# skokec/DAU-ConvNet

Measured on AMD Instinct MI355X. Metric: DAU fwd+bwd GSamples/s (N*H*W/s), higher is better.
Workload: dtype f32

## Files before the change

dau-convnet_amd/csrc/k_dense_split.hip:

```cpp
#include <algorithm>
#include <cstdint>
#include <cstdlib>
#include <type_traits>

#include "dau_tiled.hpp"

#ifndef DAU_SPLIT_R
#define DAU_SPLIT_R 3
#endif
#ifndef DAU_SPLIT_NS
#define DAU_SPLIT_NS s3
#endif

namespace dau {
namespace DAU_SPLIT_NS {

typedef _Float16 f16x8 __attribute__((ext_vector_type(8)));
typedef __attribute__((ext_vector_type(16))) float f32x16;
typedef __attribute__((ext_vector_type(4))) unsigned u32x4;
typedef __attribute__((address_space(3))) void* lds_ptr_t;
typedef __attribute__((address_space(1))) const void* glb_ptr_t;

namespace {

constexpr int kDR = DAU_SPLIT_R;
constexpr int kDK = 2 * kDR + 1;
constexpr int kDSpan = kDK - 1;
constexpr int kDTaps = kDK * kDK;
constexpr int kDRows = 8;
constexpr int kDFB = 128;
constexpr int kAhead = 2;
#ifndef DAU_SPLIT_FLUSH_TAPS
#define DAU_SPLIT_FLUSH_TAPS 0
#endif
constexpr int kFlushTaps = DAU_SPLIT_FLUSH_TAPS > 0 ? DAU_SPLIT_FLUSH_TAPS : kDK;
#ifndef DAU_SPLIT_FLUSH_ROWS
#define DAU_SPLIT_FLUSH_ROWS 4
#endif
constexpr int kFlushRows = DAU_SPLIT_FLUSH_ROWS;

inline size_t round_up(size_t v, size_t a) { return (v + a - 1) / a * a; }

struct SplitScales {
    unsigned max_w_bits;
    float sw, inv_sw;
    float pad[5];
};
__host__ __device__ __forceinline__ const float* scales_sx(const SplitScales* sc) { return reinterpret_cast<const float*>(sc + 1); }
__host__ __device__ __forceinline__ const float* scales_inv_sx(const SplitScales* sc, int N) { return reinterpret_cast<const float*>(sc + 1) + N; }
constexpr int kPartials = 1024;
inline int absmax_groups_per_image(int N, long per) {
    const long fit = std::max(1, kPartials / N), want = (per / 4 + 255) / 256 + 1;
    return (int)std::min(fit, want);
}
inline size_t scales_bytes(int N) { return sizeof(SplitScales) + (size_t)2 * N * sizeof(float); }

constexpr int kMaxSub = 4;
struct SplitGeom {
    int sub;
    int nsub_a, nb_a, nsub_b, nb_b;
    int nrb8, nrb4;
    int tall;
    int Hs, Ws, nchunk, CoutP;
    size_t hdr_bytes, xs_bytes, ws_bytes;
};

SplitGeom split_geometry(const DenseConfig& c) {
    SplitGeom g{};
    g.sub = (c.W + 7) / 8;
    const int nblocks = (g.sub + kMaxSub - 1) / kMaxSub, base = g.sub / nblocks, rem = g.sub % nblocks;
    if (rem) { g.nsub_a = base + 1; g.nb_a = rem; g.nsub_b = base; g.nb_b = nblocks - rem; }
    else { g.nsub_a = base; g.nb_a = nblocks; g.nsub_b = 0; g.nb_b = 0; }
    const int left = c.H % kDRows;
    const long wgs = (long)c.N * ((c.H + kDRows - 1) / kDRows) * nblocks * ((c.Cout + kDFB - 1) / kDFB);
    const int rows4 = DAU_TUNE_INT("DAU_SPLIT_ROWS4", 1);
    g.nrb4 = (left >= 1 && left <= 4 && rows4 != 0 && (wgs >= 1024 || rows4 == 2)) ? 1 : 0;
    g.nrb8 = c.H / kDRows + (left && !g.nrb4 ? 1 : 0);
    g.Hs = g.nrb8 * kDRows + g.nrb4 * 4 + kDSpan;
    {
        const int t4 = (c.W + 3) / 4;
        const long rows8 = (long)g.nrb8 * kDRows;
        const long flat = (long)(g.nrb4 ? rows8 + 4 : (c.H + 3) / 4 * 4) * g.sub * 8;
        const long tall = rows8 * t4 * 4 + (g.nrb4 ? 4L * g.sub * 8 : 0);
        const int want = DAU_TUNE_INT("DAU_SPLIT_TALL", 1);
        g.tall = (want != 0 && g.nrb8 > 0 && (t4 == 5 || t4 == 7) && (tall * 20 <= flat * 19 || want == 2)) ? t4 : 0;
    }
    g.Ws = g.sub * 8 + kDSpan;
    g.nchunk = (c.Cin + 15) / 16;
    g.CoutP = (int)round_up(c.Cout, kDFB);
    g.hdr_bytes = round_up(scales_bytes(c.N) + (size_t)2 * (kPartials + c.N) * sizeof(unsigned), 256);
    g.xs_bytes = round_up((size_t)c.N * g.nchunk * 4 * g.Hs * g.Ws * 16 + 4096, 256);
    g.ws_bytes = round_up(((size_t)g.nchunk * kDTaps + 8) * 2 * g.CoutP * 32, 256);
    return g;
}

constexpr int lds_pitch(int nsub) {
    int p = nsub * 8 + kDSpan;
    while (p % 16 != 8) ++p;
    return p;
}
constexpr int lds_pitch_narrow(int ntiles) {
    int p = ntiles * 4 + kDSpan;
    while (p % 16 != 4 && p % 16 != 12) ++p;
    return p;
}

}

__device__ __forceinline__ unsigned finite_bits(unsigned b) { return b < 0x7f800000u ? b : 0u; }

__device__ __forceinline__ long absmax_head(const void* p, long per, int elem_bytes, int vec_bytes) {
    const uintptr_t a = reinterpret_cast<uintptr_t>(p);
    if (a % elem_bytes) return per;
    const long head = (long)((vec_bytes - a % vec_bytes) % vec_bytes) / elem_bytes;
    return head < per ? head : per;
}

__global__ void __launch_bounds__(256) split_absmax_kernel(const float* __restrict__ in, long per, int gpi, int act, const UnitRef* __restrict__ table,
                                                           long units, unsigned* __restrict__ partial, int cap, const Guard guard) {
    if (!guard_pass(guard)) return;
    unsigned mx = 0, mw = 0;
    const int n = blockIdx.x / gpi, j = blockIdx.x - n * gpi;
    const long stride = (long)gpi * blockDim.x, t0 = j * (long)blockDim.x + threadIdx.x;
    if (act == kActF16) {
        auto wide = [](unsigned h) { return finite_bits(__float_as_uint(f16_bits_to_float(h)) & 0x7fffffffu); };
        const unsigned short* e = reinterpret_cast<const unsigned short*>(in) + n * per;
        const long head = absmax_head(e, per, 2, 8), n4 = (per - head) / 4;
        const uint2* p = reinterpret_cast<const uint2*>(e + head);
        for (long i = t0; i < n4; i += stride) {
            const uint2 v = p[i];
            mx = max(mx, max(max(wide(v.x & 0xffffu), wide(v.x >> 16)), max(wide(v.y & 0xffffu), wide(v.y >> 16))));
        }
        for (long i = t0; i < per - n4 * 4; i += stride) mx = max(mx, wide(e[i < head ? i : i + n4 * 4]));
    } else if (act == kActBF16) {
        const unsigned short* e = reinterpret_cast<const unsigned short*>(in) + n * per;
        const long head = absmax_head(e, per, 2, 8), n4 = (per - head) / 4;
        const uint2* p = reinterpret_cast<const uint2*>(e + head);
        for (long i = t0; i < n4; i += stride) {
            const uint2 v = p[i];
            mx = max(mx, max(max(finite_bits((v.x << 16) & 0x7fffffffu), finite_bits(v.x & 0x7fff0000u)),
                             max(finite_bits((v.y << 16) & 0x7fffffffu), finite_bits(v.y & 0x7fff0000u))));
        }
        for (long i = t0; i < per - n4 * 4; i += stride) mx = max(mx, finite_bits(((unsigned)e[i < head ? i : i + n4 * 4] << 16) & 0x7fffffffu));
    } else {
        const float* e = in + n * per;
        const long head = absmax_head(e, per, 4, 16), n4 = (per - head) / 4;
        const uint4* p = reinterpret_cast<const uint4*>(e + head);
        for (long i = t0; i < n4; i += stride) {
            const uint4 v = p[i];
            mx = max(mx, max(max(finite_bits(v.x & 0x7fffffffu), finite_bits(v.y & 0x7fffffffu)),
                             max(finite_bits(v.z & 0x7fffffffu), finite_bits(v.w & 0x7fffffffu))));
        }
        for (long i = t0; i < per - n4 * 4; i += stride) mx = max(mx, finite_bits(__float_as_uint(e[i < head ? i : i + n4 * 4]) & 0x7fffffffu));
    }
    for (long u = blockIdx.x * (long)blockDim.x + threadIdx.x; u < units; u += (long)gridDim.x * blockDim.x) {
        const UnitRef r = table[u];
        mw = max(mw, finite_bits(__float_as_uint(fabsf(r.w00) + fabsf(r.w01) + fabsf(r.w10) + fabsf(r.w11))));
    }
    __shared__ unsigned sx[4], sw[4];
    for (int m = 32; m >= 1; m >>= 1) { mx = max(mx, (unsigned)__shfl_xor((int)mx, m)); mw = max(mw, (unsigned)__shfl_xor((int)mw, m)); }
    if ((threadIdx.x & 63) == 0) { sx[threadIdx.x >> 6] = mx; sw[threadIdx.x >> 6] = mw; }
    __syncthreads();
    if (threadIdx.x == 0) {
        partial[blockIdx.x] = max(max(sx[0], sx[1]), max(sx[2], sx[3]));
        partial[cap + blockIdx.x] = max(max(sw[0], sw[1]), max(sw[2], sw[3]));
    }
}

__device__ __forceinline__ float limb_scale(float m) {
    if (!(m > 0.0f) || !(m < INFINITY)) return 1.0f;
    int e = ilogbf(m);
    e = 13 - e;
    e = e > 100 ? 100 : (e < -100 ? -100 : e);
    return ldexpf(1.0f, e);
}

__global__ void __launch_bounds__(256) split_scales_kernel(const unsigned* __restrict__ partial, int N, int gpi, int cap, int G,
                                                           SplitScales* __restrict__ out, const Guard guard) {
    if (!guard_pass(guard)) return;
    const int n = blockIdx.x;
    const unsigned* src = n < N ? partial + (long)n * gpi : partial + cap;
    const int cnt = n < N ? gpi : N * gpi;
    unsigned m = 0;
    for (int i = threadIdx.x; i < cnt; i += 256) m = max(m, src[i]);
    __shared__ unsigned sm[4];
    for (int k = 32; k >= 1; k >>= 1) m = max(m, (unsigned)__shfl_xor((int)m, k));
    if ((threadIdx.x & 63) == 0) sm[threadIdx.x >> 6] = m;
    __syncthreads();
    if (threadIdx.x == 0) {
        m = max(max(sm[0], sm[1]), max(sm[2], sm[3]));
        float* sx = reinterpret_cast<float*>(out + 1);
        if (n < N) {
            const float s = limb_scale(__uint_as_float(m));
            sx[n] = s; sx[N + n] = 1.0f / s;
        } else {
            const float s = limb_scale(__uint_as_float(m) * (float)G);
            out->max_w_bits = m; out->sw = s; out->inv_sw = 1.0f / s;
        }
    }
}

constexpr int kScT = 64;
__global__ void __launch_bounds__(kScT) split_densify_kernel(const UnitRef* __restrict__ table, int Cin, int G, int Cout, int CoutP, int nchunk,
                                                             const SplitScales* __restrict__ sc, _Float16* __restrict__ wsd, const Guard guard) {
    __shared__ float acc[kDTaps * kScT];
    if (!guard_pass(guard)) return;
    constexpr int FPB = kScT / 16;
    const int tid = threadIdx.x, sl = tid & 15;
    const int fq = blockIdx.x % (CoutP / FPB), chunk = blockIdx.x / (CoutP / FPB);
    const int f = fq * FPB + (tid >> 4), c = chunk * 16 + sl;
#pragma unroll 7
    for (int tap = 0; tap < kDTaps; ++tap) acc[tap * kScT + tid] = 0.0f;
    if (c < Cin && f < Cout) {
        for (int g = 0; g < G; ++g) {
            const UnitRef u = table[((long)c * G + g) * Cout + f];
            const int ty = u.oy + kDR, tx = u.ox + kDR;
            const bool y0 = ty >= 0 && ty < kDK, y1 = ty + 1 >= 0 && ty + 1 < kDK, x0 = tx >= 0 && tx < kDK, x1 = tx + 1 >= 0 && tx + 1 < kDK;
            if (y0 && x0) acc[(ty * kDK + tx) * kScT + tid] += u.w00;
            if (y0 && x1) acc[(ty * kDK + tx + 1) * kScT + tid] += u.w01;
            if (y1 && x0) acc[((ty + 1) * kDK + tx) * kScT + tid] += u.w10;
            if (y1 && x1) acc[((ty + 1) * kDK + tx + 1) * kScT + tid] += u.w11;
        }
    }
    const float sw = sc->sw;
    _Float16* dst = wsd + ((long)chunk * kDTaps * 2 * CoutP + f) * 16 + sl;
    const long limb = (long)CoutP * 16, tapstride = 2 * limb;
#pragma unroll 7
    for (int tap = 0; tap < kDTaps; ++tap) {
        const float v = acc[tap * kScT + tid] * sw;
        const _Float16 hi = (_Float16)v;
        dst[tap * tapstride] = hi;
        dst[tap * tapstride + limb] = (_Float16)(v - (float)hi);
    }
}

constexpr int kSP = 80;
struct SplitStageArgs {
    const float* in;
    const float* taps;
    const SplitScales* sc;
    _Float16* xs;
    int N, C, H, W, mirrored;
    int Hs, Ws, nchunk;
    int RB, nbands, nsegs;
    int vec;
    Guard guard;
};

__device__ __forceinline__ int fast_div(int i, int d, float inv) {
    int q = (int)(((float)i + 0.5f) * inv);
    const int r = i - q * d;
    q += (r >= d) - (r < 0);
    return q;
}

template <int K, int NCH>
__device__ __forceinline__ void split_stage_rows(float* rawl, const float* px, int col, int ch0, int wave, int nw, int lh, int ncols) {
    constexpr int kr = (K - 1) / 2;
    if (col >= ncols) return;
    float gx[K];
#pragma unroll
    for (int j = 0; j < K; ++j) gx[j] = px[j];
    for (int r = wave; r < lh; r += nw) {
        float* row = rawl + (r * 8 + ch0) * kSP + 8 + col;
        float acc[NCH];
#pragma unroll
        for (int ch = 0; ch < NCH; ++ch) {
            acc[ch] = 0.0f;
#pragma unroll
            for (int i = 0; i < K; ++i) acc[ch] = fmaf(row[ch * kSP + i - kr], gx[i], acc[ch]);
        }
#pragma unroll
        for (int ch = 0; ch < NCH; ++ch) row[ch * kSP] = acc[ch];
    }
}

template <int K, int NCH>
__device__ __forceinline__ void split_stage_walk(const float* rawl, const float* py, float sx, int col, int ch0, int ya, int yb,
                                                 int y0, int x0, int x1, int Ws, u32x4* xhi, u32x4* xlo) {
    constexpr int kr = (K - 1) / 2;
    const int x = x0 + col;
    if (x >= x1) return;
    float gy[K];
#pragma unroll
    for (int j = 0; j < K; ++j) gy[j] = py[j];
    float ring[K][NCH];
    const int nin = yb - ya + 2 * kr;
    char* dhi = reinterpret_cast<char*>(xhi + (long)kDR * Ws + kDR + x) + ch0 * 2;
    char* dlo = reinterpret_cast<char*>(xlo + (long)kDR * Ws + kDR + x) + ch0 * 2;
    for (int s0 = 0; s0 < nin; s0 += K) {
#pragma unroll
        for (int j = 0; j < K; ++j) {
            const int s = s0 + j;
            if (s < nin) {
                const float* row = rawl + ((ya - y0 + s) * 8 + ch0) * kSP + 8 + col;
#pragma unroll
                for (int ch = 0; ch < NCH; ++ch) ring[j][ch] = row[ch * kSP];
                if (s >= K - 1) {
                    typedef _Float16 f16xn __attribute__((ext_vector_type(NCH)));
                    f16xn oh, ol;
#pragma unroll
                    for (int ch = 0; ch < NCH; ++ch) {
                        float acc = 0.0f;
#pragma unroll
                        for (int i = 0; i < K; ++i) acc = fmaf(ring[(j + 1 + i) % K][ch], gy[i], acc);
                        acc *= sx;
                        const _Float16 hi = (_Float16)acc;
                        oh[ch] = hi;
                        ol[ch] = (_Float16)(acc - (float)hi);
                    }
                    const long o = (long)(ya + s - (K - 1)) * Ws * 16;
                    *reinterpret_cast<f16xn*>(dhi + o) = oh;
                    *reinterpret_cast<f16xn*>(dlo + o) = ol;
                }
            }
        }
    }
}

#ifndef DAU_SPLIT_STAGE_THREADS
#define DAU_SPLIT_STAGE_THREADS 512
#endif
constexpr int kStageThreads = DAU_SPLIT_STAGE_THREADS;
template <int KN, int A>
__global__ void __launch_bounds__(kStageThreads) split_stage_kernel(const SplitStageArgs a) {
    constexpr int K = KN & (kNhwcArg - 1);
    constexpr bool NHWC = (KN & kNhwcArg) != 0;
    extern __shared__ __attribute__((aligned(16))) float rawl[];
    if (!guard_pass(a.guard)) return;
    constexpr int kr = (K - 1) / 2;
    constexpr int PPR = kSP / 4;
    const int lane = threadIdx.x & 63, wave = threadIdx.x >> 6, nw = blockDim.x >> 6;
    int t = blockIdx.x;
    const int seg = t % a.nsegs; t /= a.nsegs;
    const int band = t % a.nbands; t /= a.nbands;
    const int grp = t % (2 * a.nchunk);
    const int n = t / (2 * a.nchunk);
    const int y0 = band * a.RB, y1 = y0 + a.RB < a.H ? y0 + a.RB : a.H;
    const int x0 = seg * 64, x1 = x0 + 64 < a.W ? x0 + 64 : a.W;
    const int lh = y1 - y0 + 2 * kr;
    const long plane = (long)a.H * a.W;
    if constexpr (NHWC) {
        constexpr int CPP = A == kActF32 ? 4 : 8, PARTS = 8 / CPP;
        const int pieces = lh * kSP * PARTS;
        constexpr int UB = (13 * 256 + kStageThreads - 1) / kStageThreads;
        for (int i0 = threadIdx.x; i0 < pieces; i0 += kStageThreads * UB) {
            float v[UB][CPP];
#pragma unroll
            for (int u = 0; u < UB; ++u) {
                const int i = i0 + u * kStageThreads, part = i % PARTS, rj = i / PARTS, r = rj / kSP, j = rj - r * kSP;
                const int c = grp * 8 + part * CPP, y = y0 - kr + r, x = x0 - 8 + j;
                const bool pix = y >= 0 && y < a.H && x >= 0 && x < a.W && i < pieces;
                if (a.vec) {
                    const bool ok = pix && c < a.C;
                    const long idx = ok ? nhwc_index(n, c, y, x, a.C, a.H, a.W) : 0;
                    if constexpr (A == kActF32) {
                        const float4 w = *reinterpret_cast<const float4*>(a.in + idx);
                        v[u][0] = mask_act(w.x, ok); v[u][1] = mask_act(w.y, ok); v[u][2] = mask_act(w.z, ok); v[u][3] = mask_act(w.w, ok);
                    } else {
                        const uint4 w = *reinterpret_cast<const uint4*>(reinterpret_cast<const unsigned short*>(a.in) + idx);
                        const unsigned q[4] = {w.x, w.y, w.z, w.w};
#pragma unroll
                        for (int k = 0; k < 4; ++k) {
                            if constexpr (A == kActF16) {
                                v[u][2 * k] = mask_act(f16_bits_to_float(q[k] & 0xffffu), ok);
                                v[u][2 * k + 1] = mask_act(f16_bits_to_float(q[k] >> 16), ok);
                            } else {
                                const unsigned m = ok ? 0xffffffffu : 0u;
                                v[u][2 * k] = __uint_as_float((q[k] << 16) & m);
                                v[u][2 * k + 1] = __uint_as_float(q[k] & 0xffff0000u & m);
                            }
                        }
                    }
                } else {
#pragma unroll
                    for (int k = 0; k < CPP; ++k) {
                        const bool ok = pix && c + k < a.C;
                        v[u][k] = mask_act(load_act_t<A>(a.in, ok ? nhwc_index(n, c + k, y, x, a.C, a.H, a.W) : 0), ok);
                    }
                }
            }
#pragma unroll
            for (int u = 0; u < UB; ++u) {
                const int i = i0 + u * kStageThreads, part = i % PARTS, rj = i / PARTS, r = rj / kSP, j = rj - r * kSP;
                if (i < pieces) {
#pragma unroll
                    for (int k = 0; k < CPP; ++k) rawl[(r * 8 + part * CPP + k) * kSP + j] = v[u][k];
                }
            }
        }
    } else
    {
        const int pieces = lh * 8 * PPR;
        constexpr int UB = (13 * 256 + kStageThreads - 1) / kStageThreads;
        for (int i0 = threadIdx.x; i0 < pieces; i0 += kStageThreads * UB) {
            float4 v[UB];
#pragma unroll
            for (int u = 0; u < UB; ++u) {
                const int i = i0 + u * kStageThreads, rc = i / PPR, q = i - rc * PPR, r = rc >> 3, ch = rc & 7;
                const int c = grp * 8 + ch, y = y0 - kr + r, xs = x0 - 8 + 4 * q;
                const bool row_in = c < a.C && y >= 0 && y < a.H && i < pieces;
                const long base = ((long)n * a.C + (c < a.C ? c : 0)) * plane;
                if (a.vec) {
                    const bool ok = row_in && xs >= 0 && xs + 4 <= a.W;
                    const long idx = base + (ok ? (long)y * a.W + xs : 0);
                    if constexpr (A == kActF16) {
                        const uint2 w = *reinterpret_cast<const uint2*>(reinterpret_cast<const unsigned short*>(a.in) + idx);
                        v[u] = make_float4(mask_act(f16_bits_to_float(w.x & 0xffffu), ok), mask_act(f16_bits_to_float(w.x >> 16), ok),
                                           mask_act(f16_bits_to_float(w.y & 0xffffu), ok), mask_act(f16_bits_to_float(w.y >> 16), ok));
                    } else if constexpr (A == kActBF16) {
                        const uint2 w = *reinterpret_cast<const uint2*>(reinterpret_cast<const unsigned short*>(a.in) + idx);
                        const unsigned m = ok ? 0xffffffffu : 0u;
                        v[u] = make_float4(__uint_as_float((w.x << 16) & m), __uint_as_float(w.x & 0xffff0000u & m),
                                           __uint_as_float((w.y << 16) & m), __uint_as_float(w.y & 0xffff0000u & m));
                    } else {
                        const float4 w = *reinterpret_cast<const float4*>(a.in + idx);
                        v[u] = make_float4(mask_act(w.x, ok), mask_act(w.y, ok), mask_act(w.z, ok), mask_act(w.w, ok));
                    }
                } else {
                    float e[4];
#pragma unroll
                    for (int k = 0; k < 4; ++k) {
                        const bool ok = row_in && xs + k >= 0 && xs + k < a.W;
                        e[k] = mask_act(load_act_t<A>(a.in, base + (ok ? (long)y * a.W + xs + k : 0)), ok);
                    }
                    v[u] = make_float4(e[0], e[1], e[2], e[3]);
                }
            }
#pragma unroll
            for (int u = 0; u < UB; ++u) {
                const int i = i0 + u * kStageThreads;
                if (i < pieces) *reinterpret_cast<float4*>(rawl + (long)i * 4) = v[u];
            }
        }
    }
    const int chunk = grp >> 1, half = grp & 1;
    const long splane = (long)a.Hs * a.Ws;
    u32x4* xhi = reinterpret_cast<u32x4*>(a.xs) + ((((long)n * a.nchunk + chunk) * 2 + 0) * 2 + half) * splane;
    u32x4* xlo = xhi + 2 * splane;
    {
        const int rs0 = band == 0 ? 0 : y0 + kDR, rs1 = band == a.nbands - 1 ? a.Hs : y1 + kDR;
        const int cs0 = seg == 0 ? 0 : x0 + kDR, cs1 = seg == a.nsegs - 1 ? a.Ws : x1 + kDR;
        const int cw = cs1 - cs0, cnt = (rs1 - rs0) * cw;
        const float inv = 1.0f / (float)cw;
        const u32x4 z = {0u, 0u, 0u, 0u};
        for (int i = threadIdx.x; i < cnt; i += blockDim.x) {
            const int rr = fast_div(i, cw, inv), r = rs0 + rr, cc = cs0 + i - rr * cw;
            if (r >= y0 + kDR && r < y1 + kDR && cc >= x0 + kDR && cc < x1 + kDR) continue;
            xhi[(long)r * a.Ws + cc] = z;
            xlo[(long)r * a.Ws + cc] = z;
        }
    }
    __syncthreads();
    const float* px = a.taps + (a.mirrored ? kTapGXR : kTapGX) * kTapPitch;
    const float* py = a.taps + (a.mirrored ? kTapGYR : kTapGY) * kTapPitch;
    if (x1 - x0 <= 32) split_stage_rows<K, 4>(rawl, px, lane & 31, (lane >> 5) * 4, wave, nw, lh, x1 - x0);
    else split_stage_rows<K, 8>(rawl, px, lane, 0, wave, nw, lh, x1 - x0);
    __syncthreads();
    const int SR = (y1 - y0 + nw - 1) / nw;
    const int ya = y0 + wave * SR, yb = ya + SR < y1 ? ya + SR : y1;
    if (ya >= yb) return;
    const float sx = scales_sx(a.sc)[n];
    if (x1 - x0 <= 32) split_stage_walk<K, 4>(rawl, py, sx, lane & 31, (lane >> 5) * 4, ya, yb, y0, x0, x1, a.Ws, xhi, xlo);
    else split_stage_walk<K, 8>(rawl, py, sx, lane, 0, ya, yb, y0, x0, x1, a.Ws, xhi, xlo);
}

struct SplitArgs {
    const _Float16* xs;
    const _Float16* wsd;
    const SplitScales* sc;
    float* out;
    const float* partial;
    int N, Cout, CoutP, H, W, Hs, Ws, nchunk, ncb, nrb, out_act;
    int col0;
    int row0;
    Guard guard;
};

constexpr int kNhwcVecOut = 0x100;
template <int NSUBN, int RG = 2, bool TT = false, bool H16 = false, bool ADD = false>
__global__ void __launch_bounds__(512) split_gather_kernel(const SplitArgs a) {
    constexpr int NSUB = NSUBN & (kNhwcArg - 1);
    constexpr bool NHWC = (NSUBN & kNhwcArg) != 0;
    static_assert(!TT || RG == 2, "tall tiles: blocks of eight rows");
    constexpr int TW = TT ? 4 : 8;
    constexpr int P = TT ? lds_pitch_narrow(NSUB) : lds_pitch(NSUB);
    constexpr int kRowsWG = 4 * RG;
    constexpr int NT0 = (RG == 2 && !TT) ? NSUB : (NSUB + 1) / 2;
    constexpr int NT1 = TT ? NSUB / 2 : NT0;
    constexpr int WR = kRowsWG + kDSpan;
    constexpr int HALF = WR * P * 16;
    constexpr int BUFU = 4 * WR * P;
    constexpr int NPIECE = (BUFU + 63) / 64;
    constexpr int BUF = NPIECE * 1024;
    constexpr int PPW = (NPIECE + 7) / 8;
    extern __shared__ __attribute__((aligned(16))) char smem[];
    if (!guard_pass(a.guard)) return;
    const int lane = threadIdx.x & 63;
    const int wave = __builtin_amdgcn_readfirstlane(threadIdx.x >> 6);
    const int fw = wave & 3, pw = wave >> 2;
    const int prow = (RG == 2 && !TT) ? 4 * pw : 0, ptile = (RG == 2 && !TT) ? 0 : pw * NT0;
    int t;
#ifdef DAU_SPLIT_NO_XCD_MAP
    t = blockIdx.x;
#else
    {
        const int nblk = gridDim.x, xcd = blockIdx.x % 8, idx = blockIdx.x / 8;
        const int per = nblk / 8, rem = nblk % 8;
        t = (xcd < rem ? xcd * (per + 1) : rem * (per + 1) + (xcd - rem) * per) + idx;
    }
#endif
    const int fb = t % (a.CoutP / kDFB); t /= (a.CoutP / kDFB);
    const int cb = t % a.ncb; t /= a.ncb;
    const int rb = t % a.nrb;
    const int n = t / a.nrb;
    const int h = lane >> 5, nn = lane & 31;

    const long xs_plane = (long)a.Hs * a.Ws;
    const int colb = a.col0 + cb * NSUB * TW;
    const int rowb = a.row0 + rb * kRowsWG;
    const u32x4* xsrc = reinterpret_cast<const u32x4*>(a.xs) + ((long)n * a.nchunk * 4) * xs_plane + (long)rowb * a.Ws + colb;
    int goff[PPW];
#pragma unroll
    for (int i = 0; i < PPW; ++i) {
        int piece = wave + 8 * i;
        piece = piece < NPIECE ? piece : NPIECE - 1;
        int L = piece * 64 + lane;
        L = L < BUFU ? L : BUFU - 1;
        const int ph = L / (WR * P), rem = L - ph * (WR * P), r = rem / P, c = rem - r * P;
        goff[i] = (int)(ph * xs_plane + (long)r * a.Ws + c);
    }
    auto issue = [&](int chunk, int buf) {
        const u32x4* src = xsrc + (long)chunk * 4 * xs_plane;
#pragma unroll
        for (int i = 0; i < PPW; ++i) {
            int piece = wave + 8 * i;
            piece = piece < NPIECE ? piece : NPIECE - 1;
            __builtin_amdgcn_global_load_lds((glb_ptr_t)(src + goff[i]), (lds_ptr_t)(smem + buf * BUF + piece * 1024), 16, 0, 0);
        }
    };

    const int prr = TT ? nn >> 2 : nn >> 3, pcc = TT ? nn & 3 : nn & 7;
    float* const out_ptr = a.out;
    const float* const part_ptr = a.partial;
    const bool out_bf16 = NHWC ? (a.out_act & 0xff) != 0 : a.out_act != 0;
    const bool vec_out = NHWC && (a.out_act & kNhwcVecOut) != 0;
    const int out_c = a.Cout, out_h = a.H, out_w = a.W;
    auto body = [&](auto ntc) __attribute__((always_inline)) {
    constexpr int NT = decltype(ntc)::value;
    f32x16 sum[NT], acc[NT];
    f32x16 zero;
#pragma unroll
    for (int i = 0; i < 16; ++i) zero[i] = 0.0f;
#pragma unroll
    for (int j = 0; j < NT; ++j) { sum[j] = zero; acc[j] = zero; }
    int rows_chained = 0;

    const f16x8* wp = reinterpret_cast<const f16x8*>(a.wsd) + ((long)(fb * kDFB + fw * 32 + nn)) * 2 + h;
    const long wlo = (long)a.CoutP * 2, wtap = 2 * wlo;
    const unsigned lane_base = (unsigned)(h * HALF + ((prow + prr) * P + ptile * TW + pcc) * 16);

#ifdef DAU_SPLIT_NO_IDLE_WAVES
    const bool live = true;
#else
    const bool live = rowb + prow < a.H && ptile < NSUB && colb + ptile * TW < a.W && fb * kDFB + fw * 32 < a.Cout;
#endif
    issue(0, 0);
    f16x8 ah[kDK], al[kDK], an[2], bn[2];
    static_assert(kAhead == 2 && kDK >= 5 && kDK <= 9, "the A ring below is written for two taps ahead");
#pragma unroll
    for (int i = 0; i < kAhead; ++i) { ah[i] = wp[i * wtap]; al[i] = wp[i * wtap + wlo]; }
    asm volatile("s_waitcnt vmcnt(0)" ::: "memory");
    __syncthreads();
    for (int chunk = 0; chunk < a.nchunk; ++chunk) {
        const int buf = chunk & 1;
        if (chunk + 1 < a.nchunk) issue(chunk + 1, buf ^ 1);
        const unsigned bbase = lane_base + buf * BUF;
#pragma unroll 1
        for (int ty = 0; ty < (live ? kDK : 0); ++ty) {
            const unsigned brow = bbase + ty * P * 16;
            f16x8 xh[NT], xl[NT];
#pragma unroll
            for (int j = 0; j < NT; ++j) xh[j] = *reinterpret_cast<const f16x8*>(smem + brow + (TW * j) * 16);
#pragma unroll
            for (int tx = 0; tx < kDK; ++tx) {
#pragma unroll
                for (int j = 0; j < NT; ++j) xl[j] = *reinterpret_cast<const f16x8*>(smem + brow + 2 * HALF + (tx + TW * j) * 16);
#pragma unroll
                for (int j = 0; j < NT; ++j) acc[j] = __builtin_amdgcn_mfma_f32_32x32x16_f16(ah[tx], xh[j], (kFlushRows == 1 && tx % kFlushTaps == 0) ? zero : acc[j], 0, 0, 0);
                if (tx + kAhead < kDK) { ah[tx + kAhead] = wp[(tx + kAhead) * wtap]; al[tx + kAhead] = wp[(tx + kAhead) * wtap + wlo]; }
                if (tx == 2 || tx == 3) { an[tx - 2] = wp[(kDK + tx - 2) * wtap]; bn[tx - 2] = wp[(kDK + tx - 2) * wtap + wlo]; }
#pragma unroll
                for (int j = 0; j < NT; ++j) acc[j] = __builtin_amdgcn_mfma_f32_32x32x16_f16(al[tx], xh[j], acc[j], 0, 0, 0);
                if (tx + 1 < kDK) {
#pragma unroll
                    for (int j = 0; j < NT; ++j) xh[j] = *reinterpret_cast<const f16x8*>(smem + brow + (tx + 1 + TW * j) * 16);
                }
#pragma unroll
                for (int j = 0; j < NT; ++j) acc[j] = __builtin_amdgcn_mfma_f32_32x32x16_f16(ah[tx], xl[j], acc[j], 0, 0, 0);
                if (tx == 0) __builtin_amdgcn_sched_group_barrier(0x100, 2 * NT, 0);
                else __builtin_amdgcn_sched_group_barrier(0x100, NT, 0);
                __builtin_amdgcn_sched_group_barrier(0x008, NT, 0);
                if (tx == 2 || tx == 3) __builtin_amdgcn_sched_group_barrier(0x020, 4, 0);
                else if (tx + kAhead < kDK) __builtin_amdgcn_sched_group_barrier(0x020, 2, 0);
                __builtin_amdgcn_sched_group_barrier(0x008, NT, 0);
                if (tx + 1 < kDK) __builtin_amdgcn_sched_group_barrier(0x100, NT, 0);
                __builtin_amdgcn_sched_group_barrier(0x008, NT, 0);
                if ((tx + 1) % kFlushTaps == 0 && tx + 1 < kDK) {
#pragma unroll
                    for (int j = 0; j < NT; ++j) sum[j] += acc[j];
                }
            }
            wp += kDK * wtap;
            ah[0] = an[0]; al[0] = bn[0]; ah[1] = an[1]; al[1] = bn[1];
            if constexpr (kFlushRows == 1) {
#pragma unroll
                for (int j = 0; j < NT; ++j) sum[j] += acc[j];
            } else {
                if (++rows_chained == kFlushRows) {
                    rows_chained = 0;
#pragma unroll
                    for (int j = 0; j < NT; ++j) { sum[j] += acc[j]; acc[j] = zero; }
                }
            }
        }
        if (chunk + 1 < a.nchunk) {
            asm volatile("s_waitcnt vmcnt(0)" ::: "memory");
            __syncthreads();
        }
    }

    if constexpr (kFlushRows > 1) {
#pragma unroll
        for (int j = 0; j < NT; ++j) sum[j] += acc[j];
    }
    const float inv_w = a.sc->inv_sw, inv_x = scales_inv_sx(a.sc, a.N)[n];
    const int y = rowb + prow + prr;
    const long plane = (long)out_h * out_w;
#pragma unroll
    for (int j = 0; j < NT; ++j) {
        const int x = colb + TW * (ptile + j) + pcc;
        if constexpr (NHWC) {
            if (y < out_h && x < out_w && ptile + j < NSUB) {
                const long pix = ((long)n * out_h + y) * out_w + x;
#pragma unroll
                for (int g4 = 0; g4 < 4; ++g4) {
                    const int f0 = fb * kDFB + fw * 32 + 8 * g4 + 4 * h;
                    float v[4];
#pragma unroll
                    for (int k = 0; k < 4; ++k) {
                        if constexpr (ADD) {
                            const int fc = f0 + k < out_c ? f0 + k : out_c - 1;
                            v[k] = sum[j][4 * g4 + k] * inv_w * inv_x + part_ptr[((long)n * out_c + fc) * plane + (long)y * out_w + x];
                        } else {
                            v[k] = sum[j][4 * g4 + k] * inv_w * inv_x;
                        }
                    }
                    const long o = pix * out_c + f0;
                    if (vec_out) {
                        if (f0 < out_c) {
                            if constexpr (H16) {
                                typedef _Float16 f16x4 __attribute__((ext_vector_type(4)));
                                *reinterpret_cast<f16x4*>(reinterpret_cast<unsigned short*>(out_ptr) + o) =
                                    f16x4{(_Float16)v[0], (_Float16)v[1], (_Float16)v[2], (_Float16)v[3]};
                            } else if (out_bf16) {
                                *reinterpret_cast<uint2*>(reinterpret_cast<unsigned short*>(out_ptr) + o) =
                                    make_uint2(bf16_bits(v[0]) | (bf16_bits(v[1]) << 16), bf16_bits(v[2]) | (bf16_bits(v[3]) << 16));
                            } else {
                                *reinterpret_cast<float4*>(out_ptr + o) = make_float4(v[0], v[1], v[2], v[3]);
                            }
                        }
                    } else {
#pragma unroll
                        for (int k = 0; k < 4; ++k) {
                            if (f0 + k < out_c) {
                                if constexpr (H16) store_act_t<kActF16>(out_ptr, o + k, v[k], false);
                                else store_act(out_ptr, o + k, v[k], out_bf16, false);
                            }
                        }
                    }
                }
            }
        } else
        if (y < out_h && x < out_w && ptile + j < NSUB) {
#pragma unroll
            for (int i = 0; i < 16; ++i) {
                const int f = fb * kDFB + fw * 32 + (i & 3) + 8 * (i >> 2) + 4 * h;
                if (f < out_c) {
                    const long o = ((long)n * out_c + f) * plane + (long)y * out_w + x;
                    if constexpr (ADD) {
                        const float v = sum[j][i] * inv_w * inv_x + part_ptr[o];
                        if constexpr (H16) store_act_t<kActF16>(out_ptr, o, v, false);
                        else store_act(out_ptr, o, v, out_bf16, false);
                    } else if constexpr (H16) store_act_t<kActF16>(out_ptr, o, sum[j][i] * inv_w * inv_x, false);
                    else store_act(out_ptr, o, sum[j][i] * inv_w * inv_x, out_bf16, false);
                }
            }
        }
    }
    };
    if constexpr (TT) {
        if (pw == 0) body(std::integral_constant<int, NT0>{});
        else body(std::integral_constant<int, NT1>{});
    } else {
        body(std::integral_constant<int, NT0>{});
    }
}

namespace {

template <int NSUB, int RG, bool TT>
constexpr size_t split_lds_bytes() { return 2 * (size_t)((4 * (4 * RG + kDSpan) * (TT ? lds_pitch_narrow(NSUB) : lds_pitch(NSUB)) + 63) / 64) * 1024; }

template <int NSUB, int RG, bool TT = false>
void launch_split(hipStream_t st, const SplitArgs* a, int grid, bool h16, bool add, bool nhwc) {
    constexpr int NH = NSUB | kNhwcArg;
    auto kern = h16 ? split_gather_kernel<NSUB, RG, TT, true> : split_gather_kernel<NSUB, RG, TT, false>;
    if (nhwc) kern = h16 ? split_gather_kernel<NH, RG, TT, true> : split_gather_kernel<NH, RG, TT, false>;
#if DAU_SPLIT_R == 3
    if (add) kern = h16 ? split_gather_kernel<NSUB, RG, TT, true, true> : split_gather_kernel<NSUB, RG, TT, false, true>;
    if (add && nhwc) kern = h16 ? split_gather_kernel<NH, RG, TT, true, true> : split_gather_kernel<NH, RG, TT, false, true>;
#endif
    if (!a) { (void)hipFuncSetAttribute(reinterpret_cast<const void*>(kern), hipFuncAttributeMaxDynamicSharedMemorySize, 160 * 1024); return; }
    constexpr size_t lds = split_lds_bytes<NSUB, RG, TT>();
    hipLaunchKernelGGL(kern, dim3(grid), dim3(512), lds, st, *a);
}

void dispatch_split(int nsub, int rg, bool h16, hipStream_t st, const SplitArgs* a, int grid, bool tall, bool add, bool nhwc) {
    if (tall) {
        if (nsub == 5) launch_split<5, 2, true>(st, a, grid, h16, add, nhwc);
        else launch_split<7, 2, true>(st, a, grid, h16, add, nhwc);
        return;
    }
    if (rg == 1) {
        switch (nsub) {
            case 1: launch_split<1, 1>(st, a, grid, h16, add, nhwc); break;
            case 2: launch_split<2, 1>(st, a, grid, h16, add, nhwc); break;
            case 3: launch_split<3, 1>(st, a, grid, h16, add, nhwc); break;
            default: launch_split<4, 1>(st, a, grid, h16, add, nhwc); break;
        }
        return;
    }
    switch (nsub) {
        case 1: launch_split<1, 2>(st, a, grid, h16, add, nhwc); break;
        case 2: launch_split<2, 2>(st, a, grid, h16, add, nhwc); break;
        case 3: launch_split<3, 2>(st, a, grid, h16, add, nhwc); break;
        default: launch_split<4, 2>(st, a, grid, h16, add, nhwc); break;
    }
}

const void* stage_for(int blur_k, int act, bool nhwc = false) {
#define DAU_SPLIT_STAGE(K) case K: if (nhwc) return act == kActF16 ? reinterpret_cast<const void*>(split_stage_kernel<K | kNhwcArg, kActF16>) : \
                                          act == kActBF16 ? reinterpret_cast<const void*>(split_stage_kernel<K | kNhwcArg, kActBF16>) : \
                                                            reinterpret_cast<const void*>(split_stage_kernel<K | kNhwcArg, kActF32>); \
                                   return act == kActF16 ? reinterpret_cast<const void*>(split_stage_kernel<K, kActF16>) : \
                                          act == kActBF16 ? reinterpret_cast<const void*>(split_stage_kernel<K, kActBF16>) : \
                                                            reinterpret_cast<const void*>(split_stage_kernel<K, kActF32>)
    switch (blur_k) {
        DAU_SPLIT_STAGE(3);
        DAU_SPLIT_STAGE(5);
        DAU_SPLIT_STAGE(7);
        DAU_SPLIT_STAGE(9);
        DAU_SPLIT_STAGE(11);
        default: return nullptr;
    }
#undef DAU_SPLIT_STAGE
}
void stage_plan(const DenseConfig& c, int* RB, int* nbands, size_t* lds) {
    const int kr = (c.blur_k - 1) / 2;
    int rows = 52 * 1024 / (8 * kSP * 4) - 2 * kr;
    const int rb = DAU_TUNE_INT("DAU_SPLIT_STAGE_RB", 0);
    if (rb > 0) rows = rb;
    rows = rows < 4 ? 4 : rows;
    const int nb = (c.H + rows - 1) / rows;
    *nbands = nb; *RB = (c.H + nb - 1) / nb;
    *lds = (size_t)(*RB + 2 * kr) * 8 * kSP * 4;
}

}

bool split_gather_configure(int N, int Cin, int Cout, int G, int H, int W, int R, int blur_k, int act, DenseConfig* cfg) {
    if (R != kDR || !stage_for(blur_k, act)) return false;
    DenseConfig c{};
    c.N = N; c.Cin = Cin; c.Cout = Cout; c.G = G; c.H = H; c.W = W; c.R = R; c.blur_k = blur_k; c.act = act;
    const SplitGeom g = split_geometry(c);
    c.nsub = g.nsub_a;
    c.ftiles = 1;
    if ((size_t)g.nchunk * 4 * g.Hs * g.Ws > (size_t)1 << 30) return false;
    *cfg = c;
    return true;
}

size_t split_gather_workspace_bytes(const DenseConfig& c) {
    const SplitGeom g = split_geometry(c);
    return g.hdr_bytes + g.xs_bytes + g.ws_bytes;
}

void split_gather_init(const DenseConfig& c) {
    const SplitGeom g = split_geometry(c);
    const bool h16 = c.act == kActF16;
    for (int rg = 1; rg <= 2; ++rg) {
        if (!(rg == 2 ? g.nrb8 : g.nrb4)) continue;
        for (int add = 0; add <= (kDR == 3 ? 1 : 0); ++add) {
            if (rg == 2 && g.tall) { dispatch_split(g.tall, 2, h16, nullptr, nullptr, 0, true, add != 0, c.nhwc != 0); continue; }
            dispatch_split(g.nsub_a, rg, h16, nullptr, nullptr, 0, false, add != 0, c.nhwc != 0);
            if (g.nb_b) dispatch_split(g.nsub_b, rg, h16, nullptr, nullptr, 0, false, add != 0, c.nhwc != 0);
        }
    }
    (void)hipFuncSetAttribute(stage_for(c.blur_k, c.act, c.nhwc != 0), hipFuncAttributeMaxDynamicSharedMemorySize, 160 * 1024);
}

void split_gather_prepare(hipStream_t st, const DenseConfig& c, const float* in, const float* filters, bool mirrored,
                          const UnitRef* table, void* workspace, const Guard& guard) {
    const SplitGeom g = split_geometry(c);
    char* ws = static_cast<char*>(workspace);
    SplitScales* sc = reinterpret_cast<SplitScales*>(ws);
    unsigned* partial = reinterpret_cast<unsigned*>(ws + scales_bytes(c.N));
    _Float16* xs = reinterpret_cast<_Float16*>(ws + g.hdr_bytes);
    _Float16* wsd = reinterpret_cast<_Float16*>(ws + g.hdr_bytes + g.xs_bytes);
    const long per = (long)c.Cin * c.H * c.W, units = (long)c.Cin * c.G * c.Cout;
    const int gpi = absmax_groups_per_image(c.N, per), cap = kPartials + c.N;
    hipLaunchKernelGGL(split_absmax_kernel, dim3(c.N * gpi), dim3(256), 0, st, in, per, gpi, c.act, table, units, partial, cap, guard);
    hipLaunchKernelGGL(split_scales_kernel, dim3(c.N + 1), dim3(256), 0, st, partial, c.N, gpi, cap, c.G, sc, guard);
    hipLaunchKernelGGL(split_densify_kernel, dim3(g.nchunk * (g.CoutP / (kScT / 16))), dim3(kScT), 0, st, table, c.Cin, c.G, c.Cout, g.CoutP,
                       g.nchunk, sc, wsd, guard);
    SplitStageArgs s{};
    s.in = in; s.taps = filters + kTaps1dOffset; s.sc = sc; s.xs = xs;
    s.N = c.N; s.C = c.Cin; s.H = c.H; s.W = c.W; s.mirrored = mirrored ? 1 : 0;
    s.Hs = g.Hs; s.Ws = g.Ws; s.nchunk = g.nchunk; s.guard = guard;
    size_t lds;
    stage_plan(c, &s.RB, &s.nbands, &lds);
    s.nsegs = (c.W + 63) / 64;
    s.vec = c.W % 4 == 0 && reinterpret_cast<uintptr_t>(in) % 16 == 0;
    if (c.nhwc) s.vec = c.Cin % (c.act == kActF32 ? 4 : 8) == 0 && reinterpret_cast<uintptr_t>(in) % 16 == 0;
    void* args[] = {&s};
    (void)hipLaunchKernel(stage_for(c.blur_k, c.act, c.nhwc != 0), dim3(c.N * 2 * g.nchunk * s.nbands * s.nsegs), dim3(kStageThreads), args, lds, st);
}

namespace {
void run_split(hipStream_t st, const DenseConfig& c, float* out, const float* partial, void* workspace, const Guard& guard) {
    const SplitGeom g = split_geometry(c);
    const bool add = partial != nullptr;
    const bool h16 = c.act == kActF16;
    char* ws = static_cast<char*>(workspace);
    SplitArgs a{};
    a.sc = reinterpret_cast<const SplitScales*>(ws);
    a.xs = reinterpret_cast<const _Float16*>(ws + g.hdr_bytes);
    a.wsd = reinterpret_cast<const _Float16*>(ws + g.hdr_bytes + g.xs_bytes);
    a.out = out; a.partial = partial;
    a.N = c.N; a.Cout = c.Cout; a.CoutP = g.CoutP; a.H = c.H; a.W = c.W; a.Hs = g.Hs; a.Ws = g.Ws; a.nchunk = g.nchunk;
    a.out_act = c.act; a.guard = guard;
    const bool nhwc = c.nhwc != 0;
    if (nhwc && c.Cout % 4 == 0 && reinterpret_cast<uintptr_t>(out) % (c.act == kActF32 ? 16 : 8) == 0) a.out_act |= kNhwcVecOut;
    for (int rg = 2; rg >= 1; --rg) {
        a.nrb = rg == 2 ? g.nrb8 : g.nrb4;
        if (!a.nrb) continue;
        a.row0 = rg == 2 ? 0 : g.nrb8 * kDRows;
        if (rg == 2 && g.tall) {
            a.ncb = 1; a.col0 = 0;
            dispatch_split(g.tall, 2, h16, st, &a, c.N * a.nrb * (g.CoutP / kDFB), true, add, nhwc);
            continue;
        }
        a.ncb = g.nb_a; a.col0 = 0;
        dispatch_split(g.nsub_a, rg, h16, st, &a, c.N * a.nrb * g.nb_a * (g.CoutP / kDFB), false, add, nhwc);
        if (g.nb_b) {
            a.ncb = g.nb_b; a.col0 = g.nb_a * g.nsub_a * 8;
            dispatch_split(g.nsub_b, rg, h16, st, &a, c.N * a.nrb * g.nb_b * (g.CoutP / kDFB), false, add, nhwc);
        }
    }
}
}

void split_gather_run(hipStream_t st, const DenseConfig& c, float* out, void* workspace, const Guard& guard) {
    run_split(st, c, out, nullptr, workspace, guard);
}

#if DAU_SPLIT_R == 3
void split_gather_run_add(hipStream_t st, const DenseConfig& c, float* out, const float* partial, void* workspace, const Guard& guard) {
    run_split(st, c, out, partial, workspace, guard);
}

SplitStaged split_gather_staged(const DenseConfig& c, const void* workspace) {
    const SplitGeom g = split_geometry(c);
    const char* ws = static_cast<const char*>(workspace);
    SplitStaged s{};
    s.sx = scales_sx(reinterpret_cast<const SplitScales*>(ws));
    s.xs = reinterpret_cast<const _Float16*>(ws + g.hdr_bytes);
    s.Hs = g.Hs; s.Ws = g.Ws; s.nchunk = g.nchunk;
    return s;
}
#endif

}
}
```

Measured before the change: 0.01674.

## Add K=32 MFMA path processing two channel chunks per pass in split gather

Adds a body32 path, on by default for R=3, that uses 16x16x32 f16 MFMA instructions. Each pass consumes two input-channel chunks, so the LDS buffers are doubled to hold chunk pairs, and weights are fetched via buffer resource loads with a two-tap-ahead register ring. The aim is fewer MFMA issues and barriers per chunk and better matrix-core utilisation. The cost is twice the LDS footprint, which may lower occupancy, plus more register pressure and hand-tuned scheduling barriers. The epilogue is factored into a shared store4 helper.

After: 0.01802 (median of 6 runs). 7.6% higher.

```diff
diff --git a/dau-convnet_amd/csrc/k_dense_split.hip b/dau-convnet_amd/csrc/k_dense_split.hip
--- a/dau-convnet_amd/csrc/k_dense_split.hip
+++ b/dau-convnet_amd/csrc/k_dense_split.hip
@@ -17,6 +17,7 @@
 
 typedef _Float16 f16x8 __attribute__((ext_vector_type(8)));
 typedef __attribute__((ext_vector_type(16))) float f32x16;
+typedef __attribute__((ext_vector_type(4))) float f32x4;
 typedef __attribute__((ext_vector_type(4))) unsigned u32x4;
 typedef __attribute__((address_space(3))) void* lds_ptr_t;
 typedef __attribute__((address_space(1))) const void* glb_ptr_t;
@@ -38,6 +39,14 @@
 #define DAU_SPLIT_FLUSH_ROWS 4
 #endif
 constexpr int kFlushRows = DAU_SPLIT_FLUSH_ROWS;
+#if !defined(DAU_SPLIT_K32)
+#if !defined(DAU_SPLIT_MFMA32) && DAU_SPLIT_R == 3
+#define DAU_SPLIT_K32 1
+#else
+#define DAU_SPLIT_K32 0
+#endif
+#endif
+constexpr bool kK32 = DAU_SPLIT_K32 != 0;
 
 inline size_t round_up(size_t v, size_t a) { return (v + a - 1) / a * a; }
 
@@ -489,10 +498,12 @@
     constexpr int NT0 = (RG == 2 && !TT) ? NSUB : (NSUB + 1) / 2;
     constexpr int NT1 = TT ? NSUB / 2 : NT0;
     constexpr int WR = kRowsWG + kDSpan;
-    constexpr int HALF = WR * P * 16;
-    constexpr int BUFU = 4 * WR * P;
+    constexpr int PLANE = kK32 ? (WR * P + 15) / 16 * 16 : WR * P;
+    constexpr int HALF = PLANE * 16;
+    constexpr int BUFU = 4 * PLANE;
     constexpr int NPIECE = (BUFU + 63) / 64;
-    constexpr int BUF = NPIECE * 1024;
+    constexpr int BUF1 = NPIECE * 1024;
+    constexpr int BUF = kK32 ? 2 * BUF1 : BUF1;
     constexpr int PPW = (NPIECE + 7) / 8;
     extern __shared__ __attribute__((aligned(16))) char smem[];
     if (!guard_pass(a.guard)) return;
@@ -527,7 +538,10 @@
         piece = piece < NPIECE ? piece : NPIECE - 1;
         int L = piece * 64 + lane;
         L = L < BUFU ? L : BUFU - 1;
-        const int ph = L / (WR * P), rem = L - ph * (WR * P), r = rem / P, c = rem - r * P;
+        const int ph = L / PLANE;
+        int rem = L - ph * PLANE;
+        rem = rem < WR * P ? rem : WR * P - 1;
+        const int r = rem / P, c = rem - r * P;
         goff[i] = (int)(ph * xs_plane + (long)r * a.Ws + c);
     }
     auto issue = [&](int chunk, int buf) {
@@ -537,6 +551,16 @@
             int piece = wave + 8 * i;
             piece = piece < NPIECE ? piece : NPIECE - 1;
             __builtin_amdgcn_global_load_lds((glb_ptr_t)(src + goff[i]), (lds_ptr_t)(smem + buf * BUF + piece * 1024), 16, 0, 0);
+        }
+        if constexpr (kK32) {
+            if (chunk + 1 < a.nchunk) {
+#pragma unroll
+                for (int i = 0; i < PPW; ++i) {
+                    int piece = wave + 8 * i;
+                    piece = piece < NPIECE ? piece : NPIECE - 1;
+                    __builtin_amdgcn_global_load_lds((glb_ptr_t)(src + 4 * xs_plane + goff[i]), (lds_ptr_t)(smem + buf * BUF + BUF1 + piece * 1024), 16, 0, 0);
+                }
+            }
         }
     };
 
@@ -546,6 +570,65 @@
     const bool out_bf16 = NHWC ? (a.out_act & 0xff) != 0 : a.out_act != 0;
     const bool vec_out = NHWC && (a.out_act & kNhwcVecOut) != 0;
     const int out_c = a.Cout, out_h = a.H, out_w = a.W;
+    auto joined = [&](float s, float inv_w, float inv_x, float part) __attribute__((always_inline)) {
+        float v = s * inv_w * inv_x + part;
+        if constexpr (H16) asm("" : "+v"(v));
+        return v;
+    };
+    auto store4 = [&](int y, int x, bool tile, int f0, const float (&s)[4], float inv_w, float inv_x) __attribute__((always_inline)) {
+        const long plane = (long)out_h * out_w;
+        if (!(y < out_h && x < out_w && tile)) return;
+        if constexpr (NHWC) {
+            const long pix = ((long)n * out_h + y) * out_w + x;
+            float v[4];
+#pragma unroll
+            for (int k = 0; k < 4; ++k) {
+                if constexpr (ADD) {
+                    const int fc = f0 + k < out_c ? f0 + k : out_c - 1;
+                    v[k] = joined(s[k], inv_w, inv_x, part_ptr[((long)n * out_c + fc) * plane + (long)y * out_w + x]);
+                } else {
+                    v[k] = s[k] * inv_w * inv_x;
+                }
+            }
+            const long o = pix * out_c + f0;
+            if (vec_out) {
+                if (f0 < out_c) {
+                    if constexpr (H16) {
+                        typedef _Float16 f16x4 __attribute__((ext_vector_type(4)));
+                        *reinterpret_cast<f16x4*>(reinterpret_cast<unsigned short*>(out_ptr) + o) =
+                            f16x4{(_Float16)v[0], (_Float16)v[1], (_Float16)v[2], (_Float16)v[3]};
+                    } else if (out_bf16) {
+                        *reinterpret_cast<uint2*>(reinterpret_cast<unsigned short*>(out_ptr) + o) =
+                            make_uint2(bf16_bits(v[0]) | (bf16_bits(v[1]) << 16), bf16_bits(v[2]) | (bf16_bits(v[3]) << 16));
+                    } else {
+                        *reinterpret_cast<float4*>(out_ptr + o) = make_float4(v[0], v[1], v[2], v[3]);
+                    }
+                }
+            } else {
+#pragma unroll
+                for (int k = 0; k < 4; ++k) {
+                    if (f0 + k < out_c) {
+                        if constexpr (H16) store_act_t<kActF16>(out_ptr, o + k, v[k], false);
+                        else store_act(out_ptr, o + k, v[k], out_bf16, false);
+                    }
+                }
+            }
+        } else {
+#pragma unroll
+            for (int k = 0; k < 4; ++k) {
+                const int f = f0 + k;
+                if (f < out_c) {
+                    const long o = ((long)n * out_c + f) * plane + (long)y * out_w + x;
+                    if constexpr (ADD) {
+                        const float v = joined(s[k], inv_w, inv_x, part_ptr[o]);
+                        if constexpr (H16) store_act_t<kActF16>(out_ptr, o, v, false);
+                        else store_act(out_ptr, o, v, out_bf16, false);
+                    } else if constexpr (H16) store_act_t<kActF16>(out_ptr, o, s[k] * inv_w * inv_x, false);
+                    else store_act(out_ptr, o, s[k] * inv_w * inv_x, out_bf16, false);
+                }
+            }
+        }
+    };
     auto body = [&](auto ntc) __attribute__((always_inline)) {
     constexpr int NT = decltype(ntc)::value;
     f32x16 sum[NT], acc[NT];
@@ -636,81 +719,160 @@
     }
     const float inv_w = a.sc->inv_sw, inv_x = scales_inv_sx(a.sc, a.N)[n];
     const int y = rowb + prow + prr;
-    const long plane = (long)out_h * out_w;
 #pragma unroll
     for (int j = 0; j < NT; ++j) {
         const int x = colb + TW * (ptile + j) + pcc;
-        if constexpr (NHWC) {
-            if (y < out_h && x < out_w && ptile + j < NSUB) {
-                const long pix = ((long)n * out_h + y) * out_w + x;
-#pragma unroll
-                for (int g4 = 0; g4 < 4; ++g4) {
-                    const int f0 = fb * kDFB + fw * 32 + 8 * g4 + 4 * h;
-                    float v[4];
-#pragma unroll
-                    for (int k = 0; k < 4; ++k) {
-                        if constexpr (ADD) {
-                            const int fc = f0 + k < out_c ? f0 + k : out_c - 1;
-                            v[k] = sum[j][4 * g4 + k] * inv_w * inv_x + part_ptr[((long)n * out_c + fc) * plane + (long)y * out_w + x];
-                        } else {
-                            v[k] = sum[j][4 * g4 + k] * inv_w * inv_x;
-                        }
+#pragma unroll
+        for (int g4 = 0; g4 < 4; ++g4) {
+            const float s4[4] = {sum[j][4 * g4], sum[j][4 * g4 + 1], sum[j][4 * g4 + 2], sum[j][4 * g4 + 3]};
+            store4(y, x, ptile + j < NSUB, fb * kDFB + fw * 32 + 8 * g4 + 4 * h, s4, inv_w, inv_x);
+        }
+    }
+    };
+    auto body32 = [&](auto ntc) __attribute__((always_inline)) {
+    constexpr int NT = decltype(ntc)::value;
+    constexpr int NG = 2 * NT;
+    constexpr int U = kDK * NG;
+    constexpr int GR = TT ? 4 : 2;
+    f32x4 sum[NG][2], acc[NG][2];
+    const f32x4 zero = {0.0f, 0.0f, 0.0f, 0.0f};
+#pragma unroll
+    for (int p = 0; p < NG; ++p) { sum[p][0] = zero; sum[p][1] = zero; acc[p][0] = zero; acc[p][1] = zero; }
+    int rows_chained = 0;
+    const int g = lane >> 4, q = lane & 15;
+    const int qr = TT ? q >> 2 : q >> 3, qc = TT ? q & 3 : q & 7;
+    const bool upper = g >= 2;
+
+    const int wlo = a.CoutP * 32, wtap = 2 * wlo;
+    const long wchunk = (long)kDTaps * wtap, wend = a.nchunk * wchunk;
+    const unsigned wlane = (unsigned)(((fb * kDFB + fw * 32 + q) * 2 + (g & 1)) * 16) + (upper ? (unsigned)wchunk : 0u);
+    auto rows_from = [&](long off) __attribute__((always_inline)) {
+        const long left = wend - off;
+        const unsigned records = left <= 0 ? 0u : left > 0xffffffffl ? 0xffffffffu : (unsigned)left;
+        return __builtin_amdgcn_make_buffer_rsrc(const_cast<char*>(reinterpret_cast<const char*>(a.wsd)) + off, 0, records, 0x00020000);
+    };
+    auto load_a = [&](__amdgpu_buffer_rsrc_t rows, int soff, int m) __attribute__((always_inline)) {
+        return __builtin_bit_cast(f16x8, __builtin_amdgcn_raw_buffer_load_b128(rows, wlane + 512 * m, soff, 0));
+    };
+    const unsigned lane_base = (unsigned)((g & 1) * HALF + ((prow + qr) * P + ptile * TW + qc) * 16);
+#ifdef DAU_SPLIT_NO_IDLE_WAVES
+    const bool live = true;
+#else
+    const bool live = rowb + prow < a.H && ptile < NSUB && colb + ptile * TW < a.W && fb * kDFB + fw * 32 < a.Cout;
+#endif
+    issue(0, 0);
+    f16x8 ah[kDK][2], al[kDK][2], an[2][2], bn[2][2];
+    static_assert(kAhead == 2 && kDK >= 5 && kDK <= 9, "the A ring below is written for two taps ahead");
+#pragma unroll
+    for (int i = 0; i < kAhead; ++i) {
+#pragma unroll
+        for (int m = 0; m < 2; ++m) { ah[i][m] = load_a(rows_from(0), i * wtap, m); al[i][m] = load_a(rows_from(0), i * wtap + wlo, m); }
+    }
+    asm volatile("s_waitcnt vmcnt(0)" ::: "memory");
+    __syncthreads();
+    const int npair = (a.nchunk + 1) >> 1;
+    for (int pair = 0; pair < npair; ++pair) {
+        const int buf = pair & 1;
+        const bool more = pair + 1 < npair;
+        if (more) issue(2 * pair + 2, buf ^ 1);
+        const bool lone = 2 * pair + 1 >= a.nchunk;
+        const unsigned bbase = lane_base + buf * BUF + (lone || !upper ? 0u : (unsigned)BUF1);
+#pragma unroll 1
+        for (int ty = 0; ty < (live ? kDK : 0); ++ty) {
+            const unsigned brow = bbase + ty * P * 16;
+            const long wrow = 2 * pair * wchunk + (long)ty * kDK * wtap;
+            const __amdgpu_buffer_rsrc_t wcur = rows_from(wrow);
+            const __amdgpu_buffer_rsrc_t wnxt = rows_from(wrow + kDK * wtap + (ty == kDK - 1 && more ? wchunk : 0));
+            f16x8 xb[3][2];
+            auto read = [&](int u, int limb) __attribute__((always_inline)) {
+                const int tx = u / NG, p = u % NG;
+                return *reinterpret_cast<const f16x8*>(smem + brow + limb * 2 * HALF + ((p & 1) * GR * P + tx + TW * (p >> 1)) * 16);
+            };
+            xb[0][0] = read(0, 0); xb[0][1] = read(0, 1); xb[1][0] = read(1, 0); xb[1][1] = read(1, 1);
+            __builtin_amdgcn_sched_group_barrier(0x100, 4, 0);
+#pragma unroll
+            for (int u = 0; u < U; ++u) {
+                const int tx = u / NG, p = u % NG;
+                if (u + 2 < U) { xb[(u + 2) % 3][0] = read(u + 2, 0); xb[(u + 2) % 3][1] = read(u + 2, 1); }
+                const f16x8 xh = xb[u % 3][0], xl = xb[u % 3][1];
+                const f16x8 h0 = ah[tx][0], h1 = ah[tx][1], l0 = al[tx][0], l1 = al[tx][1];
+                const bool fresh = kFlushRows == 1 && tx % kFlushTaps == 0;
+                acc[p][0] = __builtin_amdgcn_mfma_f32_16x16x32_f16(h0, xh, fresh ? zero : acc[p][0], 0, 0, 0);
+                acc[p][1] = __builtin_amdgcn_mfma_f32_16x16x32_f16(h1, xh, fresh ? zero : acc[p][1], 0, 0, 0);
+                if (p == 0) {
+                    if (tx + kAhead < kDK) {
+#pragma unroll
+                        for (int m = 0; m < 2; ++m) { ah[tx + kAhead][m] = load_a(wcur, (tx + kAhead) * wtap, m); al[tx + kAhead][m] = load_a(wcur, (tx + kAhead) * wtap + wlo, m); }
                     }
-                    const long o = pix * out_c + f0;
-                    if (vec_out) {
-                        if (f0 < out_c) {
-                            if constexpr (H16) {
-                                typedef _Float16 f16x4 __attribute__((ext_vector_type(4)));
-                                *reinterpret_cast<f16x4*>(reinterpret_cast<unsigned short*>(out_ptr) + o) =
-                                    f16x4{(_Float16)v[0], (_Float16)v[1], (_Float16)v[2], (_Float16)v[3]};
-                            } else if (out_bf16) {
-                                *reinterpret_cast<uint2*>(reinterpret_cast<unsigned short*>(out_ptr) + o) =
-                                    make_uint2(bf16_bits(v[0]) | (bf16_bits(v[1]) << 16), bf16_bits(v[2]) | (bf16_bits(v[3]) << 16));
-                            } else {
-                                *reinterpret_cast<float4*>(out_ptr + o) = make_float4(v[0], v[1], v[2], v[3]);
-                            }
-                        }
-                    } else {
-#pragma unroll
-                        for (int k = 0; k < 4; ++k) {
-                            if (f0 + k < out_c) {
-                                if constexpr (H16) store_act_t<kActF16>(out_ptr, o + k, v[k], false);
-                                else store_act(out_ptr, o + k, v[k], out_bf16, false);
-                            }
-                        }
+                    if (tx == kDK - 3 || tx == kDK - 2) {
+                        const int i = tx - (kDK - 3);
+#pragma unroll
+                        for (int m = 0; m < 2; ++m) { an[i][m] = load_a(wnxt, i * wtap, m); bn[i][m] = load_a(wnxt, i * wtap + wlo, m); }
                     }
                 }
-            }
-        } else
-        if (y < out_h && x < out_w && ptile + j < NSUB) {
-#pragma unroll
-            for (int i = 0; i < 16; ++i) {
-                const int f = fb * kDFB + fw * 32 + (i & 3) + 8 * (i >> 2) + 4 * h;
-                if (f < out_c) {
-                    const long o = ((long)n * out_c + f) * plane + (long)y * out_w + x;
-                    if constexpr (ADD) {
-                        const float v = sum[j][i] * inv_w * inv_x + part_ptr[o];
-                        if constexpr (H16) store_act_t<kActF16>(out_ptr, o, v, false);
-                        else store_act(out_ptr, o, v, out_bf16, false);
-                    } else if constexpr (H16) store_act_t<kActF16>(out_ptr, o, sum[j][i] * inv_w * inv_x, false);
-                    else store_act(out_ptr, o, sum[j][i] * inv_w * inv_x, out_bf16, false);
-                }
-            }
-        }
-    }
+                acc[p][0] = __builtin_amdgcn_mfma_f32_16x16x32_f16(l0, xh, acc[p][0], 0, 0, 0);
+                acc[p][1] = __builtin_amdgcn_mfma_f32_16x16x32_f16(l1, xh, acc[p][1], 0, 0, 0);
+                acc[p][0] = __builtin_amdgcn_mfma_f32_16x16x32_f16(h0, xl, acc[p][0], 0, 0, 0);
+                acc[p][1] = __builtin_amdgcn_mfma_f32_16x16x32_f16(h1, xl, acc[p][1], 0, 0, 0);
+                if (u + 2 < U) __builtin_amdgcn_sched_group_barrier(0x100, 2, 0);
+                __builtin_amdgcn_sched_group_barrier(0x008, 2, 0);
+                if (p == 0 && tx + kAhead < kDK && tx == kDK - 3) __builtin_amdgcn_sched_group_barrier(0x020, 8, 0);
+                else if (p == 0 && (tx + kAhead < kDK || tx == kDK - 2)) __builtin_amdgcn_sched_group_barrier(0x020, 4, 0);
+                __builtin_amdgcn_sched_group_barrier(0x008, 4, 0);
+                if ((tx + 1) % kFlushTaps == 0 && tx + 1 < kDK) { sum[p][0] += acc[p][0]; sum[p][1] += acc[p][1]; }
+            }
+#pragma unroll
+            for (int m = 0; m < 2; ++m) { ah[0][m] = an[0][m]; al[0][m] = bn[0][m]; ah[1][m] = an[1][m]; al[1][m] = bn[1][m]; }
+            if constexpr (kFlushRows == 1) {
+#pragma unroll
+                for (int p = 0; p < NG; ++p) { sum[p][0] += acc[p][0]; sum[p][1] += acc[p][1]; }
+            } else {
+                if (++rows_chained == kFlushRows) {
+                    rows_chained = 0;
+#pragma unroll
+                    for (int p = 0; p < NG; ++p) { sum[p][0] += acc[p][0]; sum[p][1] += acc[p][1]; acc[p][0] = zero; acc[p][1] = zero; }
+                }
+            }
+        }
+        if (more) {
+            asm volatile("s_waitcnt vmcnt(0)" ::: "memory");
+            __syncthreads();
+        }
+    }
+    if constexpr (kFlushRows > 1) {
+#pragma unroll
+        for (int p = 0; p < NG; ++p) { sum[p][0] += acc[p][0]; sum[p][1] += acc[p][1]; }
+    }
+    const float inv_w = a.sc->inv_sw, inv_x = scales_inv_sx(a.sc, a.N)[n];
+#pragma unroll
+    for (int p = 0; p < NG; ++p) {
+        const int y = rowb + prow + (p & 1) * GR + qr, x = colb + TW * (ptile + (p >> 1)) + qc;
+#pragma unroll
+        for (int m = 0; m < 2; ++m) {
+            const float s4[4] = {sum[p][m][0], sum[p][m][1], sum[p][m][2], sum[p][m][3]};
+            store4(y, x, ptile + (p >> 1) < NSUB, fb * kDFB + fw * 32 + 16 * m + 4 * g, s4, inv_w, inv_x);
+        }
+    }
+    };
+    auto run = [&](auto ntc) __attribute__((always_inline)) {
+        if constexpr (kK32) body32(ntc);
+        else body(ntc);
     };
     if constexpr (TT) {
-        if (pw == 0) body(std::integral_constant<int, NT0>{});
-        else body(std::integral_constant<int, NT1>{});
+        if (pw == 0) run(std::integral_constant<int, NT0>{});
+        else run(std::integral_constant<int, NT1>{});
     } else {
-        body(std::integral_constant<int, NT0>{});
+        run(std::integral_constant<int, NT0>{});
     }
 }
 
 namespace {
 
 template <int NSUB, int RG, bool TT>
-constexpr size_t split_lds_bytes() { return 2 * (size_t)((4 * (4 * RG + kDSpan) * (TT ? lds_pitch_narrow(NSUB) : lds_pitch(NSUB)) + 63) / 64) * 1024; }
+constexpr size_t split_lds_bytes() {
+    constexpr int plane = (4 * RG + kDSpan) * (TT ? lds_pitch_narrow(NSUB) : lds_pitch(NSUB));
+    return (kK32 ? 4 : 2) * (size_t)((4 * (kK32 ? (plane + 15) / 16 * 16 : plane) + 63) / 64) * 1024;
+}
 
 template <int NSUB, int RG, bool TT = false>
 void launch_split(hipStream_t st, const SplitArgs* a, int grid, bool h16, bool add, bool nhwc) {
```
